# lenskit/csr

Hardware: AMD Instinct MI355X
Metric: spmv_gflops (higher is better)
Workload: dtype f64

## Files before the change

csr_amd/csrc/spmv.hip:

```cpp
#include "spmv_plan.h"

#include <algorithm>
#include <ctime>

namespace csrk {
template <bool R32>
__device__ __forceinline__ double spmv_prod(double a, double x)
{
    const double t = a * x;
    return R32 ? (double)(float)t : t;
}

void free_spmv_plan(SpmvPlan *p) { delete p; }

void spmv_plan_bytes_by_part(const SpmvPlan *p, int64_t out[5])
{
    for (int i = 0; i < 5; i++) out[i] = 0;
    auto add = [&](int part, std::initializer_list<const DevBuf *> bufs) {
        for (const DevBuf *b : bufs) out[part] += (int64_t)b->bytes;
    };
    for (const AccPanel *ap : p->acc) add(0, {&ap->row_list, &ap->vals, &ap->idx, &ap->tile_row0, &ap->segs, &ap->wg_seg, &ap->partial, &ap->z, &ap->wg_map});
    const Panel &t = p->tier1;
    add(1, {&t.row_list, &t.rp, &t.ci, &t.vs, &t.tile, &t.group, &t.carry_row, &t.carry_val, &t.y, &t.crp, &t.cidx});
    const LightStream *l = &p->ls;
// ... 386 lines not shown
                int q = atomicAdd(&s_nlong, 1);
                s_long[q] = r;
                continue;
            }
            double acc = ordered_sum(s_prod, s, e);
            if (r < nr) {
                yp[i0 + r] = acc;
            } else {
                *(pt.cslot >= 0 ? yp + pt.cslot : carry_val + t) = acc;
            }
        }
        __syncthreads();
        const int nlong = s_nlong;
        for (int q = wv; q < nlong; q += PT / WAVE) {
            int r = s_long[q];
            int s = r ? s_rend[r - 1] : 0;
            int e = s_rend[r];
            double acc = 0.0;
            for (int k = s + lane; k < e; k += WAVE) acc += s_prod[k];
            acc = wave_sum(acc);
            if (lane == 0) {
                if (r < nr) {
                    yp[i0 + r] = acc;
                } else {
                    *(pt.cslot >= 0 ? yp + pt.cslot : carry_val + t) = acc;
                }
            }
        }
        pt = nx;
    }
#undef PANEL_LOAD_TILE
}

template <int CB, int PT, bool R32 = false, class SV = double, class XT = double>
__global__ __launch_bounds__(PT) void spmv_acc_kernel(const AccLaunchArgs L, const XT *__restrict__ x, int32_t ncols)
{
    uint32_t grp = 0, wg = blockIdx.x;
    if (L.wg_map) {
        const uint32_t id = L.wg_map[blockIdx.x];
        grp = id >> 16;
        wg = id & 0xffffu;
    }
    const AccGroupArgs &A = L.g[grp];
    const SV *__restrict__ pvals = (const SV *)A.vals;
    const uint16_t *__restrict__ pidx = A.idx;
    const int32_t *__restrict__ tile_row0 = A.tile_row0;
    const AccSeg *__restrict__ segs = A.segs;
    const int32_t *__restrict__ wg_seg = A.wg_seg;
    double *__restrict__ partial = A.partial;
    const int32_t H = A.H;
    const int32_t fx_g = A.fx_g;
    extern __shared__ __align__(16) unsigned char acc_smem[];
    double *s_x = (double *)acc_smem;
    double *s_acc = s_x + CB + 2;
    const int Hpad = (H + 1) & ~1;
    double *s_hval = s_acc + Hpad;
    int32_t *s_hrow = (int32_t *)(s_hval + ACC_SEG_TILES);
    constexpr int NW = PT / WAVE;
    const int tid = threadIdx.x, lane = tid & (WAVE - 1), wv = tid / WAVE;

    for (int h = tid; h < Hpad; h += PT) s_acc[h] = 0.0;
    if (tid < 2) s_x[CB + tid] = 0.0;
    const unsigned long long below = lane ? (~0ull >> (WAVE - lane)) : 0ull;
    const unsigned long long upto = below | (1ull << lane);

    int cur_blk = -1;
    const int sb = wg_seg[wg], se = wg_seg[wg + 1];
    for (int si = sb; si < se; si++) {
        const AccSeg sg = segs[si];
        if (sg.blk != cur_blk) {
            cur_blk = sg.blk;
            const int32_t w0 = sg.blk * CB;
            const int wlen = ncols - w0 < CB ? ncols - w0 : CB;
            if (wlen == CB) {
                constexpr int WL = CB / 2 / PT;
                f64x2_t v[WL];
#pragma unroll
                for (int u = 0; u < WL; u++) {
                    if (sizeof(XT) == 8) {
                        v[u] = *((const F64x2 *)(x + w0) + tid + u * PT);
                    } else {
                        const f32x2_t t = *((const F32x2 *)(x + w0) + tid + u * PT);
                        v[u].x = (double)t.x;
                        v[u].y = (double)t.y;
                    }
                }
#pragma unroll
                for (int u = 0; u < WL; u++) ((f64x2_t *)s_x)[tid + u * PT] = v[u];
            } else {
                for (int k = tid; k < wlen; k += PT) s_x[k] = (double)x[w0 + k];
            }
        }
        __syncthreads();

        const int nt = sg.ntiles;
        AccVals<SV> v, vn;
        u32x4_t ix, ixn;
        int32_t tr0 = 0, tr0n = 0;
        int t = wv;
        const int64_t pstep = (int64_t)A.n_wg;
        if (t < nt) {
            const u32x4_t *ip = (const u32x4_t *)(pidx + (sg.ptile0 + t * pstep) * ACC_TILE);
            v.load(acc_tile_at(pvals, sg.ptile0 + t * pstep), lane);
            ix = __builtin_nontemporal_load(ip + lane);
            tr0 = tile_row0[sg.tile0 + t];
        }
        for (; t < nt; t += NW) {
            const bool more = t + NW < nt;
            if (more) {
                const u32x4_t *ip = (const u32x4_t *)(pidx + (sg.ptile0 + (t + NW) * pstep) * ACC_TILE);
                vn.load(acc_tile_at(pvals, sg.ptile0 + (t + NW) * pstep), lane);
                ixn = __builtin_nontemporal_load(ip + lane);
                tr0n = tile_row0[sg.tile0 + t + NW];
            }
            uint32_t e[ACC_K] = {ix.x & 0xffffu, ix.x >> 16, ix.y & 0xffffu, ix.y >> 16,
                                 ix.z & 0xffffu, ix.z >> 16, ix.w & 0xffffu, ix.w >> 16};
            double a[ACC_K];
            if constexpr (std::is_same<SV, fix56::nib::Bytes>::value) v.get(a, fx_g, e);
            else v.get(a, fx_g);
            double xv[ACC_K];
#pragma unroll
            for (int j = 0; j < ACC_K; j++) xv[j] = s_x[e[j] & ACC_COL_MASK];
            int rw[ACC_K];
            {
                int lsum = 0;
#pragma unroll
                for (int j = 0; j < ACC_K; j++) lsum += (int)(e[j] >> ACC_ROW_SHIFT);
                int run = tr0 + wave_exscan_i32(lsum, lane);
#pragma unroll
                for (int j = 0; j < ACC_K; j++) {
                    run += (int)(e[j] >> ACC_ROW_SHIFT);
                    rw[j] = run;
                }
            }
            const int hr = rw[0];
            int cur = hr;
            double acc = 0.0, hs = 0.0;
            bool nb = false;
#pragma unroll
            for (int j = 0; j < ACC_K; j++) {
                const int r = rw[j];
                if (r != cur) {
                    if (!nb) {
                        hs = acc;
                        nb = true;
                    } else {
                        atomicAdd(&s_acc[cur], acc);
                    }
                    acc = 0.0;
                    cur = r;
                }
                if (R32) acc += spmv_prod<true>(a[j], xv[j]);
                else acc += a[j] * xv[j];
            }
            const int tr = cur;
            const double ts = acc;
            if (!nb) hs = acc;
            const int tr_prev = wave_up1_i32(tr, -1);
            const bool ne = lane > 0 && tr_prev != hr;
            const double T = wave_segscan(ts, nb || ne, lane);
            const double T_prev = wave_up1_f64(T, 0.0);
            const double X = (lane > 0 && !ne) ? T_prev : 0.0;
            const unsigned long long m_nb = __ballot(nb), m_ne = __ballot(ne);
            const bool before = ((m_nb & below) | (m_ne & upto)) != 0;
            const int ne_next = wave_down1_i32((int)ne, 1);
            const bool tail_done = lane == WAVE - 1 || ne_next != 0;
            if (nb) {
                const double hv = hs + X;
                if (before) {
                    atomicAdd(&s_acc[hr], hv);
                } else {
                    s_hrow[t] = hr;
                    s_hval[t] = hv;
                }
            }
            if (tail_done) {
                if (nb || before) {
                    atomicAdd(&s_acc[tr], T);
                } else {
                    s_hrow[t] = tr;
                    s_hval[t] = T;
                }
            }
            if (more) {
                v = vn;
                ix = ixn;
                tr0 = tr0n;
            }
        }
        __syncthreads();
        if (wv == 0) {
            for (int base = 0; base < nt; base += WAVE) {
                const int i = base + lane;
                const bool ok = i < nt;
                const int row = ok ? s_hrow[i] : -1 - lane;
                const double val = ok ? s_hval[i] : 0.0;
                const int row_prev = wave_up1_i32(row, -2 - WAVE);
                const double S = wave_segscan(val, lane == 0 || row_prev != row, lane);
                const int row_next = wave_down1_i32(row, -2 - WAVE);
                if (ok && (lane == WAVE - 1 || row_next != row)) atomicAdd(&s_acc[row], S);
            }
        }
    }
    __syncthreads();
    for (int h = tid; h < H; h += PT) partial[(int64_t)wg * H + h] = s_acc[h];
}

struct EpiJob {
    int32_t kind, blocks;
    const int32_t *carry_row;
    const double *carry_val;
    int64_t n;
    double *fy;
    const double *partial;
    const int32_t *row_list;
    int32_t H, n_wg, G;
    int32_t extra;
    const int32_t *crp, *cidx;
    const double *cval;
};
struct EpiJobs {
    EpiJob j[6];
    int32_t n;
};
constexpr int EPI_THREADS = 1024;

__global__ __launch_bounds__(EPI_THREADS) void spmv_epilogue_kernel(EpiJobs jobs, double *__restrict__ y)
{
    __shared__ double s_p[EPI_THREADS / WAVE][WAVE];
    int b = blockIdx.x, q = 0;
    while (q + 1 < jobs.n && b >= jobs.j[q].blocks) b -= jobs.j[q++].blocks;
    const EpiJob &J = jobs.j[q];
    if (J.kind == 0) {
        const int64_t t = (int64_t)b * EPI_THREADS + threadIdx.x;
// ... 412 lines not shown
    int32_t c[LS_STAGE_IPT], d[LS_STAGE_IPT];
#pragma unroll
    for (int q = 0; q < LS_STAGE_IPT; q++) {
        const int32_t k = k0 + (int32_t)threadIdx.x + q * LS_STAGE_THREADS;
        c[q] = k < k1 ? (int32_t)__builtin_nontemporal_load(a_col + k) : -1;
        d[q] = k < k1 ? __builtin_nontemporal_load(a_dst + k) : 0;
    }
    for (int i = threadIdx.x; i < W; i += LS_STAGE_THREADS) s_x[i] = c0 + i < ncols ? (double)x[c0 + i] : 0.0;
    __syncthreads();
    for (int32_t kb = k0; kb < k1; kb += LS_STAGE_THREADS * LS_STAGE_IPT) {
        int32_t cn[LS_STAGE_IPT], dn[LS_STAGE_IPT];
        const int32_t kn = kb + LS_STAGE_THREADS * LS_STAGE_IPT;
        if (kn < k1) {
#pragma unroll
            for (int q = 0; q < LS_STAGE_IPT; q++) {
                const int32_t k = kn + (int32_t)threadIdx.x + q * LS_STAGE_THREADS;
                cn[q] = k < k1 ? (int32_t)__builtin_nontemporal_load(a_col + k) : -1;
                dn[q] = k < k1 ? __builtin_nontemporal_load(a_dst + k) : 0;
            }
        }
#pragma unroll
        for (int q = 0; q < LS_STAGE_IPT; q++)
            if (c[q] >= 0) xg[d[q]] = s_x[c[q]];
        if (kn < k1) {
#pragma unroll
            for (int q = 0; q < LS_STAGE_IPT; q++) c[q] = cn[q], d[q] = dn[q];
        }
    }
}

int spmv_kernel_attributes()
{
    for (const void *f : {(const void *)spmv_acc_kernel<ACC_CB, ACC_THREADS>, (const void *)spmv_lstream_kernel<LS_PLAIN>,
                          (const void *)spmv_lstream_kernel<LS_RND>, (const void *)spmv_lstream_kernel<LS_PLAIN, true>,
                          (const void *)spmv_lstream_kernel<LS_RND, true>, (const void *)spmv_acc_kernel<ACC_CB, ACC_THREADS, true>,
                          (const void *)spmv_lstream_kernel<LS_PLAIN, false, true>, (const void *)spmv_lstream_kernel<LS_RND, false, true>,
                          (const void *)spmv_lstream_kernel<LS_PLAIN, true, true>, (const void *)spmv_lstream_kernel<LS_RND, true, true>,
                          (const void *)spmv_acc_kernel<ACC_CB, ACC_THREADS, false, float>,
                          (const void *)spmv_acc_kernel<ACC_CB, ACC_THREADS, true, float>,
                          (const void *)spmv_lstream_kernel<LS_PLAIN, false, false, float>, (const void *)spmv_lstream_kernel<LS_RND, false, false, float>,
                          (const void *)spmv_lstream_kernel<LS_PLAIN, true, false, float>, (const void *)spmv_lstream_kernel<LS_RND, true, false, float>,
                          (const void *)spmv_lstream_kernel<LS_PLAIN, false, true, float>, (const void *)spmv_lstream_kernel<LS_RND, false, true, float>,
                          (const void *)spmv_lstream_kernel<LS_PLAIN, true, true, float>, (const void *)spmv_lstream_kernel<LS_RND, true, true, float>,
                          (const void *)spmv_lstream_kernel<LS_RND24>, (const void *)spmv_lstream_kernel<LS_RND24, true>,
                          (const void *)spmv_lstream_kernel<LS_RND24, false, true>, (const void *)spmv_lstream_kernel<LS_RND24, true, true>,
                          (const void *)spmv_lstream_kernel<LS_RND24, false, false, float>, (const void *)spmv_lstream_kernel<LS_RND24, true, false, float>,
                          (const void *)spmv_lstream_kernel<LS_RND24, false, true, float>, (const void *)spmv_lstream_kernel<LS_RND24, true, true, float>,
                          (const void *)spmv_acc_kernel<ACC_CB, ACC_THREADS, false, double, float>,
                          (const void *)spmv_acc_kernel<ACC_CB, ACC_THREADS, true, double, float>,
                          (const void *)spmv_acc_kernel<ACC_CB, ACC_THREADS, false, float, float>,
                          (const void *)spmv_acc_kernel<ACC_CB, ACC_THREADS, true, float, float>,
                          (const void *)spmv_acc_kernel<ACC_CB, ACC_THREADS, false, fix56::Packed>,
                          (const void *)spmv_acc_kernel<ACC_CB, ACC_THREADS, true, fix56::Packed>,
                          (const void *)spmv_acc_kernel<ACC_CB, ACC_THREADS, false, fix56::Packed, float>,
                          (const void *)spmv_acc_kernel<ACC_CB, ACC_THREADS, true, fix56::Packed, float>,
                          (const void *)spmv_acc_kernel<ACC_CB, ACC_THREADS, false, fix56::nib::Bytes>,
                          (const void *)spmv_acc_kernel<ACC_CB, ACC_THREADS, true, fix56::nib::Bytes>,
                          (const void *)spmv_acc_kernel<ACC_CB, ACC_THREADS, false, fix56::nib::Bytes, float>,
                          (const void *)spmv_acc_kernel<ACC_CB, ACC_THREADS, true, fix56::nib::Bytes, float>})
        CSRK_HIP(hipFuncSetAttribute(f, hipFuncAttributeMaxDynamicSharedMemorySize, (int)(160 * 1024)));
    CSRK_HIP(hipFuncSetAttribute((const void *)ls_stage_kernel<double>, hipFuncAttributeMaxDynamicSharedMemorySize, (int)(LS_STAGE_WMAX * 8)));
    CSRK_HIP(hipFuncSetAttribute((const void *)ls_stage_kernel<float>, hipFuncAttributeMaxDynamicSharedMemorySize, (int)(LS_STAGE_WMAX * 8)));
    return CSRK_OK;
}

static int get_plan_locked(Matrix *m, hipStream_t s, SpmvPlan **out, bool launching)
{
    if (launching) m->spmv_calls++;
    const char *env = getenv("CSRK_SPMV_HEAVY_SPLIT"), *env_hot = getenv("CSRK_SPMV_HOT"), *env_ls = getenv("CSRK_SPMV_STREAM");
    const bool eager = (env && env[0] == '1') || (env_hot && env_hot[0] == '1') || (env_ls && env_ls[0] == '1') || !launching;
    const bool want_split = eager || m->spmv_calls >= 2;
    if (m->spmv_plan && !m->spmv_plan->split_considered && want_split && m->spmv_plan->algo == CSRK_SPMV_MERGE &&
        !m->spmv_plan->profiling) {
        if (hipDeviceSynchronize() != hipSuccess) {
            set_error("device synchronisation failed: %s", hipGetErrorString(hipGetLastError()));
            return CSRK_ERR_HIP;
        }
        free_spmv_plan(m->spmv_plan);
        m->spmv_plan = nullptr;
    }
    if (!m->spmv_plan) {
        SpmvPlan *p = new (std::nothrow) SpmvPlan();
        CSRK_REQUIRE(p, "out of host memory");
        p->algo = m->spmv_algo == CSRK_SPMV_AUTO ? CSRK_SPMV_MERGE : m->spmv_algo;
        (void)s;
        int rc = build_spmv_plan(m, p, want_split);
        if (rc == CSRK_OK && hipDeviceSynchronize() != hipSuccess) {
            set_error("SpMV plan construction failed: %s", hipGetErrorString(hipGetLastError()));
            rc = CSRK_ERR_HIP;
        }
        if (rc != CSRK_OK) {
            delete p;
// ... 70 lines not shown
            KernelTimer ks(p, s, 3);
            const unsigned gs = (unsigned)(ceil_div(p->ls.n_stage_blk, 8) * 8);
            ls_stage_kernel<XT><<<gs, LS_STAGE_THREADS, (size_t)p->ls.stage_w * 8, s>>>(
                d_x, m->ncols, p->ls.stage_w, p->ls.a_col.as<uint16_t>(), p->ls.a_dst.as<int32_t>(),
                p->ls.blk_start.as<int32_t>(), p->ls.n_stage_blk, p->ls.xg.as<double>());
            ks.stop();
            CSRK_LAUNCH_CHECK();
        }
        if (do_light && p->n_hot && !(p->ls.on && p->ls.n_cold)) {
            hot_pack_kernel<XT><<<(unsigned)ceil_div(p->n_hot, 256), 256, 0, s>>>(d_x, p->hot_cols.as<int32_t>(), p->n_hot,
                                                                            p->xh.as<double>());
            CSRK_LAUNCH_CHECK();
        }
        bool t0_rides = false;
        if (do_heavy && p->n_heavy && !p->acc.empty()) {
            KernelTimer kh(p, s, 1);
            for (size_t a0 = 0; a0 < p->acc.size(); a0 += (size_t)p->acc[a0]->launch_groups) {
                AccPanel *ap = p->acc[a0];
                const int gb = ap->launch_groups;
                if (gb < 1 || gb > accgroups::MAX_GROUPS || a0 + (size_t)gb > p->acc.size()) {
                    set_error("internal: tier 0's groups and launches disagree");
                    return CSRK_ERR_INVALID;
                }
                AccLaunchArgs L = {};
                size_t lds = 0;
                for (int g = 0; g < gb; g++) {
                    const AccPanel *aq = p->acc[a0 + (size_t)g];
                    L.g[g] = {aq->vals.p, aq->idx.as<uint16_t>(), aq->tile_row0.as<int32_t>(), aq->segs.as<AccSeg>(),
                              aq->wg_seg.as<int32_t>(), aq->partial.as<double>(), aq->nrow, aq->n_wg, aq->fx_g, 0};
                    lds = aq->lds > lds ? aq->lds : lds;
                }
                L.wg_map = gb > 1 ? ap->wg_map.as<uint32_t>() : nullptr;
                const unsigned n_blocks = (unsigned)(gb > 1 ? ap->launch_wgs : ap->n_wg);
#define ACC_LAUNCH(SV) spmv_acc_kernel<ACC_CB, ACC_THREADS, R32, SV, XT><<<n_blocks, ACC_THREADS, lds, s>>>(L, d_x, m->ncols)
                if (ap->f32) ACC_LAUNCH(float);
                else if (ap->nib) ACC_LAUNCH(fix56::nib::Bytes);
                else if (ap->fix56) ACC_LAUNCH(fix56::Packed);
                else ACC_LAUNCH(double);
#undef ACC_LAUNCH
                CSRK_LAUNCH_CHECK();
            }
            kh.stop();
        }
        if (do_heavy && p->n_heavy && p->tier1.on) {
            Panel *pn = &p->tier1;
            KernelTimer kh(p, s, 2);
#define PANEL_ARGS(PP)                                                                                              \
    pn->rp.as<PP>(), pn->ci.as<int32_t>(), pn->vs.as<double>(), d_x, m->ncols, pn->y.as<double>(),                    \
        pn->tile.as<PanelTile>(), pn->group.as<PanelGroup>(), pn->rows, pn->carry_row.as<int32_t>(),                  \
        pn->carry_val.as<double>(), pn->nnz, pn->cb, rider
            PanelRider rider = {};
            rider.first = pn->groups;
            for (int q = 0; q < accgroups::MAX_GROUPS; q++) rider.start[q] = INT32_MAX;
            int64_t rider_wgs = 0;
            if (PANEL_T1 / WAVE == 4 && do_heavy && !p->acc.empty() && (size_t)p->acc[0]->launch_groups == p->acc.size() &&
                p->acc.size() <= (size_t)accgroups::MAX_GROUPS && p->acc[0]->z.p) {
                for (size_t q = 0; q < p->acc.size(); q++) {
                    AccPanel *ap = p->acc[q];
                    rider.partial[q] = ap->partial.as<double>();
                    rider.z[q] = ap->z.as<double>();
                    rider.H[q] = ap->nrow;
                    rider.n_wg[q] = ap->n_wg;
                    rider.start[q] = (int32_t)rider_wgs;
                    rider_wgs += ceil_div(ap->nrow, WAVE);
                }
                t0_rides = true;
            }
// ... 436 lines not shown
        a_tiles += ap->tiles;
        a_rows += ap->nrow;
        a_nnz += ap->nnz;
        a_nb = ap->nb;
    }
    const bool af = !p->acc.empty();
    const int64_t plan_bytes = spmv_plan_bytes(p);
    int64_t part[5];
    spmv_plan_bytes_by_part(p, part);
    const int64_t v[34] = {p->algo == CSRK_SPMV_MERGE ? p->n_tiles : p->n_segs,
                           p->algo == CSRK_SPMV_MERGE ? p->tile_items : VEC_SEG,
                           p->n_heavy, p->algo == CSRK_SPMV_MERGE ? p->nnz_light : m->nnz,
                           a_tiles, a_nb, p->heavy_min, af ? ACC_CB : 0, p->n_heavy ? 2 : 0, a_rows, a_nnz,
                           t1.nrow, t1.rows, t1.nnz, p->tier1_min, t1.cb,
                           p->n_hot, (int64_t)(p->hot_cover * 1e6), af ? 1 : 0, p->hot_slots,
                           p->ls.on ? 1 : 0, p->ls.n_tiles, p->ls.n_runs, p->ls.grid, p->ls.n_cold, plan_bytes,
                           p->ls.round_start.p ? p->ls.stage_tiles : 0,
                           a_wgs, 0, part[0], part[1], part[2], part[3], part[4]};
    for (int i = 0; i < n && i < 34; i++) out[i] = v[i];
    const LightStream &ls = p->ls;
    const bool rnd = ls.on && ls.n_cold && ls.round_start.p;
    const int64_t plain_rounds = ls.on ? ceil_div(ls.n_tiles, LS_THREADS / WAVE) : 0;
    const int64_t w[8] = {ls.on && ls.dense ? 1 : 0,
                          ls.on && ls.idx24 ? 1 : 0,
                          ls.on ? p->n_hot_lds : 0,
                          rnd ? ls.n_rounds : plain_rounds,
                          rnd ? ls.max_wg_rounds : (ls.on ? ceil_div(plain_rounds, (int64_t)ls.grid) : 0),
                          rnd ? ls.n_stage_blk : 0,
                          rnd ? ls.stage_w : 0,
                          ls.on && ls.f32 ? 1 : 0};
    for (int i = 34; i < n && i < 42; i++) out[i] = w[i - 34];
    const int64_t u[6] = {t1.nb, t1.tiles, t1.ncs, t1.listed, t1.groups, t1.pad_groups};
    for (int i = 42; i < n && i < 48; i++) out[i] = u[i - 42];
    return CSRK_OK;
}

int csrk_spmv_stream_limits(int64_t *out, int n)
{
    CSRK_REQUIRE(out && n >= 0, "out is NULL");
    const int64_t v[13] = {ACC_TILE, ACC_K, LS_THREADS / WAVE, LS_SEQ, LS_RID, LS_HOT_LDS, LS_RND_HOT, LS_RND_CAP, LS_RND_MAXTILES,
                           LS_STAGE_WMAX, LS_STAGE_THREADS * LS_STAGE_IPT, TIERB_MIN_DEFAULT, HOT_SLOTS_MAX};
    for (int i = 0; i < n && i < 13; i++) out[i] = v[i];
    return CSRK_OK;
}


int csrk_spmv_plan_info(csrk_handle_t h, int64_t *n_tiles, int32_t *tile_items)
{
    Matrix *m = from_handle(h);
    if (!m) return CSRK_ERR_INVALID;
    SpmvPlan *p = nullptr;
    CSRK_TRY(get_plan(m, nullptr, &p));
    if (n_tiles) *n_tiles = p->algo == CSRK_SPMV_MERGE ? p->n_tiles : p->n_segs;
    if (tile_items) *tile_items = p->algo == CSRK_SPMV_MERGE ? p->tile_items : VEC_SEG;
    return CSRK_OK;
}

}
```

csr_amd/csrc/spmv_plan.h:

```cpp
#pragma once
#include "common.h"
#include "device_loads.h"
#include "wave.h"
#include "fix56.h"
#include "acc_groups.h"

#include <type_traits>
#include <vector>

namespace csrk {

__device__ __forceinline__ double wave_sum(double v)
{
#pragma unroll
    for (int off = WAVE / 2; off > 0; off >>= 1) v += __shfl_down(v, off, WAVE);
    return v;
}

__device__ __forceinline__ double ordered_sum(const double *p, int s, int e)
{
    double acc = 0.0;
    int k = s;
    for (; k + 4 <= e; k += 4) {
        const double a = p[k], b = p[k + 1], c = p[k + 2], d = p[k + 3];
        acc += a;
        acc += b;
        acc += c;
        acc += d;
    }
    for (; k < e; k++) acc += p[k];
    return acc;
}

struct Panel {
    bool on = false, p64 = false;
    int32_t cb = 0, nb = 0, nrow = 0;
    int64_t rows = 0, tiles = 0, nnz = 0, groups = 0;
    DevBuf row_list;
    DevBuf rp, ci, vs, tile, group, carry_row, carry_val, y;
    int32_t ncs = 0;
    DevBuf crp, cidx;
    int64_t listed = 0, pad_groups = 0;
};

struct AccSeg {
    int64_t tile0;
    int64_t ptile0;
    int32_t ntiles;
    int32_t blk;
};

struct AccPanel {
    int32_t nrow = 0, nb = 0, n_wg = 0;
    int32_t launch_groups = 1, launch_wgs = 0;
    DevBuf wg_map;
    int64_t tiles = 0, nnz = 0, n_segs = 0;
    size_t lds = 0;
    DevBuf row_list, vals, idx, tile_row0, segs, wg_seg, partial;
    DevBuf z;
    bool f32 = false;
    bool fix56 = false;
    bool nib = false;
    int32_t fx_g = 0;
};

struct LightStream {
    bool on = false;
    int64_t n_tiles = 0;
    int32_t n_runs = 0, n_out = 0;
    unsigned grid = 0;
    DevBuf vals, idx, rowids, tile_base, carry_row, carry_val;
    bool idx24 = false;
    bool f32 = false;
    bool dense = false;
    int64_t n_cold = 0;
    int32_t n_stage_blk = 0, stage_w = 0;
    DevBuf xg, a_col, a_dst, blk_start;
    int32_t stage_tiles = 0;
    int32_t n_rounds = 0, max_wg_rounds = 0;
    DevBuf round_start, round_tile0, wg_round0;
};

struct SpmvPlan {
    int algo = CSRK_SPMV_MERGE;
    int tile_items = 0;
    int64_t n_tiles = 0;
    DevBuf tile_row;
    DevBuf carry_row;
    DevBuf carry_val;
// ... 289 lines not shown
```

csr_amd/csrc/spmv_plan.hip:

```cpp
#include "spmv_plan.h"

#include <algorithm>
#include <cstring>
#include <ctime>
#include <type_traits>

namespace csrk {
struct PlanTrace {
    bool on;
    double t0;
    static double now()
    {
        timespec ts;
        clock_gettime(CLOCK_MONOTONIC, &ts);
        return ts.tv_sec * 1e3 + ts.tv_nsec * 1e-6;
    }
    PlanTrace() : on(getenv("CSRK_PLAN_TRACE") != nullptr), t0(0.0)
    {
        if (on) {
            (void)hipDeviceSynchronize();
            t0 = now();
        }
    }
    void lap(const char *what)
// ... 941 lines not shown
        }
    const int64_t n_tasks = (int64_t)trow.size();
    CSRK_TRY(pstart.alloc((size_t)(pairs + n) * 4));
    CSRK_TRY(d_trow.alloc((size_t)(n_tasks ? n_tasks : 1) * 4));
    CSRK_TRY(d_tpiece.alloc((size_t)(n_tasks ? n_tasks : 1) * 4));
    CSRK_TRY(stage_h2d(d_trow.p, trow.data(), (size_t)n_tasks * 4, s));
    CSRK_TRY(stage_h2d(d_tpiece.p, tpiece.data(), (size_t)n_tasks * 4, s));
    acc_pairstart_kernel<P><<<(unsigned)(ceil_div(ceil_div(n_tasks * WAVE, 256), 8) * 8), 256, 0, s>>>(
        rp, m->d_colinds, ap->row_list.as<int32_t>(), n, nb, ACC_CB, d_trow.as<int32_t>(), d_tpiece.as<int32_t>(), n_tasks,
        pstart.as<int32_t>());
    CSRK_LAUNCH_CHECK();
    tr.lap("  tier 0: pair starts");
    acc_paircount_kernel<<<(unsigned)ceil_div(pairs, 256), 256, 0, s>>>(pstart.as<int32_t>(), pairs, n, off.as<int64_t>());
    CSRK_LAUNCH_CHECK();
    DevBuf gap;
    CSRK_TRY(gap.alloc((size_t)pairs * 4));
    acc_gap_kernel<<<(unsigned)ceil_div((int64_t)nb * WAVE, 256), 256, 0, s>>>(off.as<int64_t>(), n, nb, gap.as<int32_t>());
    CSRK_LAUNCH_CHECK();
    CSRK_TRY(exclusive_scan_i64(off.as<int64_t>(), off.as<int64_t>(), pairs, s));
    CSRK_TRY(bends.alloc((size_t)(nb + 1) * 8));
    panel_blockends_kernel<<<(unsigned)ceil_div(nb + 1, 256), 256, 0, s>>>(off.as<int64_t>(), n, nb, bends.as<int64_t>());
    CSRK_LAUNCH_CHECK();
    std::vector<int64_t> be((size_t)nb + 1), t0((size_t)nb + 1);
    CSRK_TRY(stage_d2h(be.data(), bends.p, (size_t)(nb + 1) * 8, s));
    CSRK_HIP(hipStreamSynchronize(s));
    t0[0] = 0;
    for (int32_t b = 0; b < nb; b++) t0[b + 1] = t0[b] + ceil_div(be[b + 1] - be[b], ACC_TILE);
    const int64_t n_tiles = t0[nb];
    CSRK_TRY(stage_h2d(bends.p, t0.data(), (size_t)(nb + 1) * 8, s));
    tr.lap("  tier 0: counts, gaps, scan");
    int cus = 0;
    CSRK_HIP(hipDeviceGetAttribute(&cus, hipDeviceAttributeMultiprocessorCount, m->device));
    int64_t n_wg = wg_want > 0 ? wg_want : cus > 0 ? cus : 256;
    if (n_wg > n_tiles) n_wg = n_tiles;
    if (n_wg < 1) n_wg = 1;
    std::vector<int64_t> wg_t0((size_t)n_wg + 1);
    int64_t share_max = 0;
    for (int64_t w = 0; w <= n_wg; w++) wg_t0[(size_t)w] = n_tiles * w / n_wg;
    for (int64_t w = 0; w < n_wg; w++) share_max = std::max(share_max, wg_t0[(size_t)w + 1] - wg_t0[(size_t)w]);
    const int64_t n_phys = share_max * n_wg;
    DevBuf d_wg_t0;
    CSRK_TRY(d_wg_t0.alloc((size_t)(n_wg + 1) * 8));
    CSRK_TRY(stage_h2d(d_wg_t0.p, wg_t0.data(), (size_t)(n_wg + 1) * 8, s));
    ap->f32 = VT == CSRK_VAL_F32;
    DevBuf fx;
    CSRK_TRY(fx.alloc(16));
    if (VT == CSRK_VAL_F64 && n > 0 && form != ACC_FORM_RAW) {
        const char *env = getenv("CSRK_SPMV_FIX56");
        if (!(env && env[0] == '0')) {
            int32_t h[4] = {0, INT32_MAX, INT32_MIN, 0};
            CSRK_TRY(stage_h2d(fx.p, h, sizeof h, s));
            acc_range_kernel<P><<<dim3((unsigned)n, 16), 256, 0, s>>>(rp, (const double *)m->d_values, ap->row_list.as<int32_t>(),
                                                                     fx.as<int32_t>());
            CSRK_LAUNCH_CHECK();
            CSRK_TRY(stage_d2h(h, fx.p, sizeof h, s));
            CSRK_HIP(hipStreamSynchronize(s));
            fix56::Range r;
            r.bad = h[0];
            r.lo = h[1];
            r.hi = h[2];
            ap->fix56 = fix56::packable(r, ap->fx_g);
            ap->nib = ap->fix56 && form == ACC_FORM_NIB;
            tr.lap("  tier 0: value grid test");
        }
    }
    CSRK_TRY(ap->idx.alloc((size_t)n_phys * ACC_TILE * 2));
// ... 48 lines not shown
    for (int64_t w = 0; w < n_wg; w++) {
        wg_seg[(size_t)w] = (int32_t)segs.size();
        int64_t t = wg_t0[(size_t)w];
        const int64_t t_end = wg_t0[(size_t)w + 1];
        while (t < t_end) {
            while (t0[b + 1] <= t) b++;
            int64_t e = t_end < t0[b + 1] ? t_end : t0[b + 1];
            if (e - t > ACC_SEG_TILES) e = t + ACC_SEG_TILES;
            AccSeg sg;
            sg.tile0 = t;
            sg.ptile0 = (t - wg_t0[(size_t)w]) * n_wg + w;
            sg.ntiles = (int32_t)(e - t);
            sg.blk = b;
            segs.push_back(sg);
            t = e;
        }
    }
    wg_seg[(size_t)n_wg] = (int32_t)segs.size();
    CSRK_TRY(ap->segs.alloc(segs.size() * sizeof(AccSeg)));
    CSRK_TRY(ap->wg_seg.alloc(wg_seg.size() * 4));
    CSRK_TRY(stage_h2d(ap->segs.p, segs.data(), segs.size() * sizeof(AccSeg), s));
    CSRK_TRY(stage_h2d(ap->wg_seg.p, wg_seg.data(), wg_seg.size() * 4, s));
    CSRK_TRY(ap->partial.alloc((size_t)n_wg * n * 8));
    CSRK_TRY(ap->z.alloc((size_t)n * 8));
    ap->lds = (size_t)(ACC_CB + 2) * 8 + (size_t)((n + 1) & ~1) * 8 + (size_t)ACC_SEG_TILES * 12;
    CSRK_TRY(spmv_kernel_attributes());
    CSRK_HIP(hipStreamSynchronize(s));
    ap->nrow = n;
    ap->nb = nb;
    ap->n_wg = (int32_t)n_wg;
    ap->tiles = n_tiles;
    ap->nnz = nnz_rows;
    ap->n_segs = (int64_t)segs.size();
    if (tr.on)
        fprintf(stderr, "[csrk plan]   tier 0 group: rows %d entries %lld workgroups %lld tiles %lld, %.1f per segment%s\n", n,
                (long long)nnz_rows, (long long)n_wg, (long long)n_tiles, segs.empty() ? 0.0 : (double)n_tiles / (double)segs.size(),
                ap->nib ? " (nib)" : ap->fix56 ? " (fix56)" : ap->f32 ? " (float32)" : " (raw)");
    tr.lap("  tier 0: segments");
    return CSRK_OK;
}

static int acc_nib_knob()
{
    const char *env = getenv("CSRK_SPMV_NIB");
    if (!env || !env[0]) return -1;
    return env[0] == '0' ? 0 : 1;
}

static int acc_groups_knob()
{
    const char *e = getenv("CSRK_ACC_GROUPS");
    const int g = e ? atoi(e) : ACC_GROUPS_DEFAULT;
    return g < 1 ? 1 : g > accgroups::MAX_GROUPS ? accgroups::MAX_GROUPS : g;
}
static int32_t acc_group_rows_knob()
{
    const char *e = getenv("CSRK_ACC_GROUP_ROWS");
    const int r = e ? atoi(e) : ACC_MAXROWS;
    return r < 1 || r > ACC_MAXROWS ? ACC_MAXROWS : r;
}


template <class P>
static int build_heavy_split(Matrix *m, SpmvPlan *p, hipStream_t s, bool allow_tier1 = true)
{
    p->n_heavy = 0;
// ... 840 lines not shown
```

Baseline: 835.6.

## Pipeline tile and x-window prefetch across segments in accumulate SpMV kernel

Adds a pipelined variant of the accumulate kernel that prefetches the next segment's first tile and the next x window into registers while the current segment is still being reduced. Segment descriptors are read through a uniform (scalar) address space. This is meant to hide the global-load latency at segment boundaries that the old loop exposed after each barrier. The variant is on by default behind an env switch. It adds register pressure from holding the staged x window and doubles the number of template instantiations.

```diff
diff --git a/csr_amd/csrc/spmv.hip b/csr_amd/csrc/spmv.hip
--- a/csr_amd/csrc/spmv.hip
+++ b/csr_amd/csrc/spmv.hip
@@ -442,7 +442,97 @@
 #undef PANEL_LOAD_TILE
 }
 
-template <int CB, int PT, bool R32 = false, class SV = double, class XT = double>
+template <bool R32, class SV>
+__device__ __forceinline__ void acc_tile_reduce(const AccVals<SV> &v, const u32x4_t ix, const int tr0, const int32_t fx_g,
+                                                const double *s_x, double *s_acc, int32_t *s_hrow, double *s_hval, const int t,
+                                                const int lane, const unsigned long long below, const unsigned long long upto)
+{
+    uint32_t e[ACC_K] = {ix.x & 0xffffu, ix.x >> 16, ix.y & 0xffffu, ix.y >> 16,
+                         ix.z & 0xffffu, ix.z >> 16, ix.w & 0xffffu, ix.w >> 16};
+    double a[ACC_K];
+    if constexpr (std::is_same<SV, fix56::nib::Bytes>::value) v.get(a, fx_g, e);
+    else v.get(a, fx_g);
+    double xv[ACC_K];
+#pragma unroll
+    for (int j = 0; j < ACC_K; j++) xv[j] = s_x[e[j] & ACC_COL_MASK];
+    int rw[ACC_K];
+    {
+        int lsum = 0;
+#pragma unroll
+        for (int j = 0; j < ACC_K; j++) lsum += (int)(e[j] >> ACC_ROW_SHIFT);
+        int run = tr0 + wave_exscan_i32(lsum, lane);
+#pragma unroll
+        for (int j = 0; j < ACC_K; j++) {
+            run += (int)(e[j] >> ACC_ROW_SHIFT);
+            rw[j] = run;
+        }
+    }
+    const int hr = rw[0];
+    int cur = hr;
+    double acc = 0.0, hs = 0.0;
+    bool nb = false;
+#pragma unroll
+    for (int j = 0; j < ACC_K; j++) {
+        const int r = rw[j];
+        if (r != cur) {
+            if (!nb) {
+                hs = acc;
+                nb = true;
+            } else {
+                atomicAdd(&s_acc[cur], acc);
+            }
+            acc = 0.0;
+            cur = r;
+        }
+        if (R32) acc += spmv_prod<true>(a[j], xv[j]);
+        else acc += a[j] * xv[j];
+    }
+    const int tr = cur;
+    const double ts = acc;
+    if (!nb) hs = acc;
+    const int tr_prev = wave_up1_i32(tr, -1);
+    const bool ne = lane > 0 && tr_prev != hr;
+    const double T = wave_segscan(ts, nb || ne, lane);
+    const double T_prev = wave_up1_f64(T, 0.0);
+    const double X = (lane > 0 && !ne) ? T_prev : 0.0;
+    const unsigned long long m_nb = __ballot(nb), m_ne = __ballot(ne);
+    const bool before = ((m_nb & below) | (m_ne & upto)) != 0;
+    const int ne_next = wave_down1_i32((int)ne, 1);
+    const bool tail_done = lane == WAVE - 1 || ne_next != 0;
+    if (nb) {
+        const double hv = hs + X;
+        if (before) {
+            atomicAdd(&s_acc[hr], hv);
+        } else {
+            s_hrow[t] = hr;
+            s_hval[t] = hv;
+        }
+    }
+    if (tail_done) {
+        if (nb || before) {
+            atomicAdd(&s_acc[tr], T);
+        } else {
+            s_hrow[t] = tr;
+            s_hval[t] = T;
+        }
+    }
+}
+
+__device__ __forceinline__ AccSeg acc_seg_uniform(const AccSeg *segs, int i)
+{
+    typedef const int64_t __attribute__((address_space(4))) *C64;
+    typedef const int32_t __attribute__((address_space(4))) *C32;
+    static_assert(sizeof(AccSeg) == 24, "two 64-bit words, two 32-bit words");
+    const uintptr_t at = (uintptr_t)(segs + i);
+    AccSeg sg;
+    sg.tile0 = ((C64)at)[0];
+    sg.ptile0 = ((C64)at)[1];
+    sg.ntiles = ((C32)at)[4];
+    sg.blk = ((C32)at)[5];
+    return sg;
+}
+
+template <int CB, int PT, bool R32 = false, class SV = double, class XT = double, bool PIPE = false>
 __global__ __launch_bounds__(PT) void spmv_acc_kernel(const AccLaunchArgs L, const XT *__restrict__ x, int32_t ncols)
 {
     uint32_t grp = 0, wg = blockIdx.x;
@@ -474,142 +564,164 @@
     const unsigned long long below = lane ? (~0ull >> (WAVE - lane)) : 0ull;
     const unsigned long long upto = below | (1ull << lane);
 
-    int cur_blk = -1;
-    const int sb = wg_seg[wg], se = wg_seg[wg + 1];
-    for (int si = sb; si < se; si++) {
-        const AccSeg sg = segs[si];
-        if (sg.blk != cur_blk) {
-            cur_blk = sg.blk;
-            const int32_t w0 = sg.blk * CB;
+    auto fold_heads = [&](const int nt) {
+        for (int base = 0; base < nt; base += WAVE) {
+            const int i = base + lane;
+            const bool ok = i < nt;
+            const int row = ok ? s_hrow[i] : -1 - lane;
+            const double val = ok ? s_hval[i] : 0.0;
+            const int row_prev = wave_up1_i32(row, -2 - WAVE);
+            const double S = wave_segscan(val, lane == 0 || row_prev != row, lane);
+            const int row_next = wave_down1_i32(row, -2 - WAVE);
+            if (ok && (lane == WAVE - 1 || row_next != row)) atomicAdd(&s_acc[row], S);
+        }
+    };
+    if constexpr (PIPE) {
+        const int wvu = __builtin_amdgcn_readfirstlane(wv);
+        const int sb = __builtin_amdgcn_readfirstlane(wg_seg[wg]), se = __builtin_amdgcn_readfirstlane(wg_seg[wg + 1]);
+        const int64_t pstep = (int64_t)A.n_wg;
+        constexpr int WL = CB / 2 / PT;
+        static_assert(WL * 2 * PT == CB, "a window is WL pairs per thread");
+        typedef typename std::conditional<sizeof(XT) == 8, f64x2_t, f32x2_t>::type X2;
+        typedef typename std::conditional<sizeof(XT) == 8, F64x2, F32x2>::type X2U;
+        X2 wr[WL];
+        auto window_request = [&](const int blk) {
+            const int32_t w0 = blk * CB;
             const int wlen = ncols - w0 < CB ? ncols - w0 : CB;
             if (wlen == CB) {
-                constexpr int WL = CB / 2 / PT;
-                f64x2_t v[WL];
+#pragma unroll
+                for (int u = 0; u < WL; u++) wr[u] = *((const X2U *)(x + w0) + tid + u * PT);
+            } else {
 #pragma unroll
                 for (int u = 0; u < WL; u++) {
-                    if (sizeof(XT) == 8) {
-                        v[u] = *((const F64x2 *)(x + w0) + tid + u * PT);
-                    } else {
-                        const f32x2_t t = *((const F32x2 *)(x + w0) + tid + u * PT);
-                        v[u].x = (double)t.x;
-                        v[u].y = (double)t.y;
+                    const int k0 = tid + 2 * u * PT, k1 = k0 + PT;
+                    wr[u].x = x[w0 + (k0 < wlen ? k0 : wlen - 1)];
+                    wr[u].y = x[w0 + (k1 < wlen ? k1 : wlen - 1)];
+                }
+            }
+        };
+        auto window_store = [&](const int blk) {
+            const int32_t w0 = blk * CB;
+            const int wlen = ncols - w0 < CB ? ncols - w0 : CB;
+            if (wlen == CB) {
+#pragma unroll
+                for (int u = 0; u < WL; u++) {
+                    f64x2_t d;
+                    d.x = (double)wr[u].x;
+                    d.y = (double)wr[u].y;
+                    ((f64x2_t *)s_x)[tid + u * PT] = d;
+                }
+            } else {
+#pragma unroll
+                for (int u = 0; u < WL; u++) {
+                    const int k0 = tid + 2 * u * PT, k1 = k0 + PT;
+                    if (k0 < wlen) s_x[k0] = (double)wr[u].x;
+                    if (k1 < wlen) s_x[k1] = (double)wr[u].y;
+                }
+            }
+        };
+        AccVals<SV> v, vn;
+        u32x4_t ix = {0, 0, 0, 0}, ixn;
+        int32_t tr0 = 0, tr0n;
+        auto tile_request = [&](AccVals<SV> &dv, u32x4_t &dix, int32_t &dtr, const int64_t ptile, const int64_t ltile) {
+            dv.load(acc_tile_at(pvals, ptile), lane);
+            dix = __builtin_nontemporal_load((const u32x4_t *)(pidx + ptile * ACC_TILE) + lane);
+            dtr = tile_row0[ltile];
+        };
+        if (sb < se) {
+            AccSeg sg = acc_seg_uniform(segs, sb);
+            window_request(sg.blk);
+            if (wvu < sg.ntiles) tile_request(v, ix, tr0, sg.ptile0 + wvu * pstep, sg.tile0 + wvu);
+            bool fill = true;
+            for (int si = sb; si < se; si++) {
+                const bool has_next = si + 1 < se;
+                const AccSeg nx = acc_seg_uniform(segs, has_next ? si + 1 : si);
+                if (fill) window_store(sg.blk);
+                __syncthreads();
+                const int nt = sg.ntiles;
+                const bool next_mine = has_next && wvu < nx.ntiles;
+                const int64_t pt_first = nx.ptile0 + wvu * pstep, lt_first = nx.tile0 + wvu;
+                const bool fill_next = has_next && nx.blk != sg.blk;
+                if (wvu >= nt) {
+                    if (next_mine) tile_request(v, ix, tr0, pt_first, lt_first);
+                    if (fill_next) window_request(nx.blk);
+                }
+                for (int t = wvu; t < nt; t += NW) {
+                    const bool more = t + NW < nt;
+                    const int64_t pt_n = more ? sg.ptile0 + (t + NW) * pstep : next_mine ? pt_first : sg.ptile0 + t * pstep;
+                    const int64_t lt_n = more ? sg.tile0 + t + NW : next_mine ? lt_first : sg.tile0 + t;
+                    tile_request(vn, ixn, tr0n, pt_n, lt_n);
+                    if (!more && fill_next) window_request(nx.blk);
+                    acc_tile_reduce<R32, SV>(v, ix, tr0, fx_g, s_x, s_acc, s_hrow, s_hval, t, lane, below, upto);
+                    v = vn;
+                    ix = ixn;
+                    tr0 = tr0n;
+                }
+                __syncthreads();
+                if (wv == 0) fold_heads(nt);
+                fill = fill_next;
+                sg = nx;
+            }
+        }
+    } else {
+        int cur_blk = -1;
+        const int sb = wg_seg[wg], se = wg_seg[wg + 1];
+        for (int si = sb; si < se; si++) {
+            const AccSeg sg = segs[si];
+            if (sg.blk != cur_blk) {
+                cur_blk = sg.blk;
+                const int32_t w0 = sg.blk * CB;
+                const int wlen = ncols - w0 < CB ? ncols - w0 : CB;
+                if (wlen == CB) {
+                    constexpr int WL = CB / 2 / PT;
+                    f64x2_t v[WL];
+#pragma unroll
+                    for (int u = 0; u < WL; u++) {
+                        if (sizeof(XT) == 8) {
+                            v[u] = *((const F64x2 *)(x + w0) + tid + u * PT);
+                        } else {
+                            const f32x2_t t = *((const F32x2 *)(x + w0) + tid + u * PT);
+                            v[u].x = (double)t.x;
+                            v[u].y = (double)t.y;
+                        }
                     }
+#pragma unroll
+                    for (int u = 0; u < WL; u++) ((f64x2_t *)s_x)[tid + u * PT] = v[u];
+                } else {
+                    for (int k = tid; k < wlen; k += PT) s_x[k] = (double)x[w0 + k];
                 }
-#pragma unroll
-                for (int u = 0; u < WL; u++) ((f64x2_t *)s_x)[tid + u * PT] = v[u];
-            } else {
-                for (int k = tid; k < wlen; k += PT) s_x[k] = (double)x[w0 + k];
-            }
-        }
-        __syncthreads();
-
-        const int nt = sg.ntiles;
-        AccVals<SV> v, vn;
-        u32x4_t ix, ixn;
-        int32_t tr0 = 0, tr0n = 0;
-        int t = wv;
-        const int64_t pstep = (int64_t)A.n_wg;
-        if (t < nt) {
-            const u32x4_t *ip = (const u32x4_t *)(pidx + (sg.ptile0 + t * pstep) * ACC_TILE);
-            v.load(acc_tile_at(pvals, sg.ptile0 + t * pstep), lane);
-            ix = __builtin_nontemporal_load(ip + lane);
-            tr0 = tile_row0[sg.tile0 + t];
-        }
-        for (; t < nt; t += NW) {
-            const bool more = t + NW < nt;
-            if (more) {
-                const u32x4_t *ip = (const u32x4_t *)(pidx + (sg.ptile0 + (t + NW) * pstep) * ACC_TILE);
-                vn.load(acc_tile_at(pvals, sg.ptile0 + (t + NW) * pstep), lane);
-                ixn = __builtin_nontemporal_load(ip + lane);
-                tr0n = tile_row0[sg.tile0 + t + NW];
-            }
-            uint32_t e[ACC_K] = {ix.x & 0xffffu, ix.x >> 16, ix.y & 0xffffu, ix.y >> 16,
-                                 ix.z & 0xffffu, ix.z >> 16, ix.w & 0xffffu, ix.w >> 16};
-            double a[ACC_K];
-            if constexpr (std::is_same<SV, fix56::nib::Bytes>::value) v.get(a, fx_g, e);
-            else v.get(a, fx_g);
-            double xv[ACC_K];
-#pragma unroll
-            for (int j = 0; j < ACC_K; j++) xv[j] = s_x[e[j] & ACC_COL_MASK];
-            int rw[ACC_K];
-            {
-                int lsum = 0;
-#pragma unroll
-                for (int j = 0; j < ACC_K; j++) lsum += (int)(e[j] >> ACC_ROW_SHIFT);
-                int run = tr0 + wave_exscan_i32(lsum, lane);
-#pragma unroll
-                for (int j = 0; j < ACC_K; j++) {
-                    run += (int)(e[j] >> ACC_ROW_SHIFT);
-                    rw[j] = run;
+            }
+            __syncthreads();
+
+            const int nt = sg.ntiles;
+            AccVals<SV> v, vn;
+            u32x4_t ix, ixn;
+            int32_t tr0 = 0, tr0n = 0;
+            int t = wv;
+            const int64_t pstep = (int64_t)A.n_wg;
+            if (t < nt) {
+                const u32x4_t *ip = (const u32x4_t *)(pidx + (sg.ptile0 + t * pstep) * ACC_TILE);
+                v.load(acc_tile_at(pvals, sg.ptile0 + t * pstep), lane);
+                ix = __builtin_nontemporal_load(ip + lane);
+                tr0 = tile_row0[sg.tile0 + t];
+            }
+            for (; t < nt; t += NW) {
+                const bool more = t + NW < nt;
+                if (more) {
+                    const u32x4_t *ip = (const u32x4_t *)(pidx + (sg.ptile0 + (t + NW) * pstep) * ACC_TILE);
+                    vn.load(acc_tile_at(pvals, sg.ptile0 + (t + NW) * pstep), lane);
+                    ixn = __builtin_nontemporal_load(ip + lane);
+                    tr0n = tile_row0[sg.tile0 + t + NW];
                 }
-            }
-            const int hr = rw[0];
-            int cur = hr;
-            double acc = 0.0, hs = 0.0;
-            bool nb = false;
-#pragma unroll
-            for (int j = 0; j < ACC_K; j++) {
-                const int r = rw[j];
-                if (r != cur) {
-                    if (!nb) {
-                        hs = acc;
-                        nb = true;
-                    } else {
-                        atomicAdd(&s_acc[cur], acc);
-                    }
-                    acc = 0.0;
-                    cur = r;
+                acc_tile_reduce<R32, SV>(v, ix, tr0, fx_g, s_x, s_acc, s_hrow, s_hval, t, lane, below, upto);
+                if (more) {
+                    v = vn;
+                    ix = ixn;
+                    tr0 = tr0n;
                 }
-                if (R32) acc += spmv_prod<true>(a[j], xv[j]);
-                else acc += a[j] * xv[j];
-            }
-            const int tr = cur;
-            const double ts = acc;
-            if (!nb) hs = acc;
-            const int tr_prev = wave_up1_i32(tr, -1);
-            const bool ne = lane > 0 && tr_prev != hr;
-            const double T = wave_segscan(ts, nb || ne, lane);
-            const double T_prev = wave_up1_f64(T, 0.0);
-            const double X = (lane > 0 && !ne) ? T_prev : 0.0;
-            const unsigned long long m_nb = __ballot(nb), m_ne = __ballot(ne);
-            const bool before = ((m_nb & below) | (m_ne & upto)) != 0;
-            const int ne_next = wave_down1_i32((int)ne, 1);
-            const bool tail_done = lane == WAVE - 1 || ne_next != 0;
-            if (nb) {
-                const double hv = hs + X;
-                if (before) {
-                    atomicAdd(&s_acc[hr], hv);
-                } else {
-                    s_hrow[t] = hr;
-                    s_hval[t] = hv;
-                }
-            }
-            if (tail_done) {
-                if (nb || before) {
-                    atomicAdd(&s_acc[tr], T);
-                } else {
-                    s_hrow[t] = tr;
-                    s_hval[t] = T;
-                }
-            }
-            if (more) {
-                v = vn;
-                ix = ixn;
-                tr0 = tr0n;
-            }
-        }
-        __syncthreads();
-        if (wv == 0) {
-            for (int base = 0; base < nt; base += WAVE) {
-                const int i = base + lane;
-                const bool ok = i < nt;
-                const int row = ok ? s_hrow[i] : -1 - lane;
-                const double val = ok ? s_hval[i] : 0.0;
-                const int row_prev = wave_up1_i32(row, -2 - WAVE);
-                const double S = wave_segscan(val, lane == 0 || row_prev != row, lane);
-                const int row_next = wave_down1_i32(row, -2 - WAVE);
-                if (ok && (lane == WAVE - 1 || row_next != row)) atomicAdd(&s_acc[row], S);
-            }
+            }
+            __syncthreads();
+            if (wv == 0) fold_heads(nt);
         }
     }
     __syncthreads();
@@ -1088,12 +1200,16 @@
 int spmv_kernel_attributes()
 {
     for (const void *f : {(const void *)spmv_acc_kernel<ACC_CB, ACC_THREADS>, (const void *)spmv_lstream_kernel<LS_PLAIN>,
+                          (const void *)spmv_acc_kernel<ACC_CB, ACC_THREADS, false, double, double, true>,
+                          (const void *)spmv_acc_kernel<ACC_CB, ACC_THREADS, true, double, double, true>,
                           (const void *)spmv_lstream_kernel<LS_RND>, (const void *)spmv_lstream_kernel<LS_PLAIN, true>,
                           (const void *)spmv_lstream_kernel<LS_RND, true>, (const void *)spmv_acc_kernel<ACC_CB, ACC_THREADS, true>,
                           (const void *)spmv_lstream_kernel<LS_PLAIN, false, true>, (const void *)spmv_lstream_kernel<LS_RND, false, true>,
                           (const void *)spmv_lstream_kernel<LS_PLAIN, true, true>, (const void *)spmv_lstream_kernel<LS_RND, true, true>,
                           (const void *)spmv_acc_kernel<ACC_CB, ACC_THREADS, false, float>,
+                          (const void *)spmv_acc_kernel<ACC_CB, ACC_THREADS, false, float, double, true>,
                           (const void *)spmv_acc_kernel<ACC_CB, ACC_THREADS, true, float>,
+                          (const void *)spmv_acc_kernel<ACC_CB, ACC_THREADS, true, float, double, true>,
                           (const void *)spmv_lstream_kernel<LS_PLAIN, false, false, float>, (const void *)spmv_lstream_kernel<LS_RND, false, false, float>,
                           (const void *)spmv_lstream_kernel<LS_PLAIN, true, false, float>, (const void *)spmv_lstream_kernel<LS_RND, true, false, float>,
                           (const void *)spmv_lstream_kernel<LS_PLAIN, false, true, float>, (const void *)spmv_lstream_kernel<LS_RND, false, true, float>,
@@ -1103,17 +1219,29 @@
                           (const void *)spmv_lstream_kernel<LS_RND24, false, false, float>, (const void *)spmv_lstream_kernel<LS_RND24, true, false, float>,
                           (const void *)spmv_lstream_kernel<LS_RND24, false, true, float>, (const void *)spmv_lstream_kernel<LS_RND24, true, true, float>,
                           (const void *)spmv_acc_kernel<ACC_CB, ACC_THREADS, false, double, float>,
+                          (const void *)spmv_acc_kernel<ACC_CB, ACC_THREADS, false, double, float, true>,
                           (const void *)spmv_acc_kernel<ACC_CB, ACC_THREADS, true, double, float>,
+                          (const void *)spmv_acc_kernel<ACC_CB, ACC_THREADS, true, double, float, true>,
                           (const void *)spmv_acc_kernel<ACC_CB, ACC_THREADS, false, float, float>,
+                          (const void *)spmv_acc_kernel<ACC_CB, ACC_THREADS, false, float, float, true>,
                           (const void *)spmv_acc_kernel<ACC_CB, ACC_THREADS, true, float, float>,
+                          (const void *)spmv_acc_kernel<ACC_CB, ACC_THREADS, true, float, float, true>,
                           (const void *)spmv_acc_kernel<ACC_CB, ACC_THREADS, false, fix56::Packed>,
+                          (const void *)spmv_acc_kernel<ACC_CB, ACC_THREADS, false, fix56::Packed, double, true>,
                           (const void *)spmv_acc_kernel<ACC_CB, ACC_THREADS, true, fix56::Packed>,
+                          (const void *)spmv_acc_kernel<ACC_CB, ACC_THREADS, true, fix56::Packed, double, true>,
                           (const void *)spmv_acc_kernel<ACC_CB, ACC_THREADS, false, fix56::Packed, float>,
+                          (const void *)spmv_acc_kernel<ACC_CB, ACC_THREADS, false, fix56::Packed, float, true>,
                           (const void *)spmv_acc_kernel<ACC_CB, ACC_THREADS, true, fix56::Packed, float>,
+                          (const void *)spmv_acc_kernel<ACC_CB, ACC_THREADS, true, fix56::Packed, float, true>,
                           (const void *)spmv_acc_kernel<ACC_CB, ACC_THREADS, false, fix56::nib::Bytes>,
+                          (const void *)spmv_acc_kernel<ACC_CB, ACC_THREADS, false, fix56::nib::Bytes, double, true>,
                           (const void *)spmv_acc_kernel<ACC_CB, ACC_THREADS, true, fix56::nib::Bytes>,
+                          (const void *)spmv_acc_kernel<ACC_CB, ACC_THREADS, true, fix56::nib::Bytes, double, true>,
                           (const void *)spmv_acc_kernel<ACC_CB, ACC_THREADS, false, fix56::nib::Bytes, float>,
-                          (const void *)spmv_acc_kernel<ACC_CB, ACC_THREADS, true, fix56::nib::Bytes, float>})
+                          (const void *)spmv_acc_kernel<ACC_CB, ACC_THREADS, false, fix56::nib::Bytes, float, true>,
+                          (const void *)spmv_acc_kernel<ACC_CB, ACC_THREADS, true, fix56::nib::Bytes, float>,
+                          (const void *)spmv_acc_kernel<ACC_CB, ACC_THREADS, true, fix56::nib::Bytes, float, true>})
         CSRK_HIP(hipFuncSetAttribute(f, hipFuncAttributeMaxDynamicSharedMemorySize, (int)(160 * 1024)));
     CSRK_HIP(hipFuncSetAttribute((const void *)ls_stage_kernel<double>, hipFuncAttributeMaxDynamicSharedMemorySize, (int)(LS_STAGE_WMAX * 8)));
     CSRK_HIP(hipFuncSetAttribute((const void *)ls_stage_kernel<float>, hipFuncAttributeMaxDynamicSharedMemorySize, (int)(LS_STAGE_WMAX * 8)));
@@ -1250,7 +1378,11 @@
                 }
                 L.wg_map = gb > 1 ? ap->wg_map.as<uint32_t>() : nullptr;
                 const unsigned n_blocks = (unsigned)(gb > 1 ? ap->launch_wgs : ap->n_wg);
-#define ACC_LAUNCH(SV) spmv_acc_kernel<ACC_CB, ACC_THREADS, R32, SV, XT><<<n_blocks, ACC_THREADS, lds, s>>>(L, d_x, m->ncols)
+#define ACC_LAUNCH(SV)                                                                                                       \
+    do {                                                                                                                     \
+        if (ap->pipe) spmv_acc_kernel<ACC_CB, ACC_THREADS, R32, SV, XT, true><<<n_blocks, ACC_THREADS, lds, s>>>(L, d_x, m->ncols); \
+        else spmv_acc_kernel<ACC_CB, ACC_THREADS, R32, SV, XT, false><<<n_blocks, ACC_THREADS, lds, s>>>(L, d_x, m->ncols);  \
+    } while (0)
                 if (ap->f32) ACC_LAUNCH(float);
                 else if (ap->nib) ACC_LAUNCH(fix56::nib::Bytes);
                 else if (ap->fix56) ACC_LAUNCH(fix56::Packed);
@@ -1753,6 +1885,14 @@
     for (int i = 34; i < n && i < 42; i++) out[i] = w[i - 34];
     const int64_t u[6] = {t1.nb, t1.tiles, t1.ncs, t1.listed, t1.groups, t1.pad_groups};
     for (int i = 42; i < n && i < 48; i++) out[i] = u[i - 42];
+    int64_t a_segs = 0, a_wg_segs = 0, a_min_tiles = 0;
+    for (const AccPanel *ap : p->acc) {
+        if (ap->n_segs) a_min_tiles = a_segs ? std::min<int64_t>(a_min_tiles, ap->min_seg_tiles) : ap->min_seg_tiles;
+        a_segs += ap->n_segs;
+        a_wg_segs = std::max<int64_t>(a_wg_segs, ap->max_wg_segs);
+    }
+    const int64_t sg3[3] = {a_segs, a_wg_segs, a_min_tiles};
+    for (int i = 48; i < n && i < 51; i++) out[i] = sg3[i - 48];
     return CSRK_OK;
 }
 
diff --git a/csr_amd/csrc/spmv_plan.h b/csr_amd/csrc/spmv_plan.h
--- a/csr_amd/csrc/spmv_plan.h
+++ b/csr_amd/csrc/spmv_plan.h
@@ -55,6 +55,8 @@
     int32_t launch_groups = 1, launch_wgs = 0;
     DevBuf wg_map;
     int64_t tiles = 0, nnz = 0, n_segs = 0;
+    int32_t max_wg_segs = 0, min_seg_tiles = 0;
+    bool pipe = true;
     size_t lds = 0;
     DevBuf row_list, vals, idx, tile_row0, segs, wg_seg, partial;
     DevBuf z;
diff --git a/csr_amd/csrc/spmv_plan.hip b/csr_amd/csrc/spmv_plan.hip
--- a/csr_amd/csrc/spmv_plan.hip
+++ b/csr_amd/csrc/spmv_plan.hip
@@ -997,6 +997,8 @@
     int cus = 0;
     CSRK_HIP(hipDeviceGetAttribute(&cus, hipDeviceAttributeMultiprocessorCount, m->device));
     int64_t n_wg = wg_want > 0 ? wg_want : cus > 0 ? cus : 256;
+    if (const char *e = getenv("CSRK_ACC_WGS"))
+        if (atoi(e) > 0 && n_wg > atoi(e)) n_wg = atoi(e);
     if (n_wg > n_tiles) n_wg = n_tiles;
     if (n_wg < 1) n_wg = 1;
     std::vector<int64_t> wg_t0((size_t)n_wg + 1);
@@ -1111,6 +1113,14 @@
     ap->tiles = n_tiles;
     ap->nnz = nnz_rows;
     ap->n_segs = (int64_t)segs.size();
+    ap->max_wg_segs = 0;
+    for (int64_t w = 0; w < n_wg; w++) ap->max_wg_segs = std::max(ap->max_wg_segs, wg_seg[(size_t)w + 1] - wg_seg[(size_t)w]);
+    ap->min_seg_tiles = segs.empty() ? 0 : INT32_MAX;
+    for (const AccSeg &sg : segs) ap->min_seg_tiles = std::min(ap->min_seg_tiles, sg.ntiles);
+    {
+        const char *env = getenv("CSRK_SPMV_ACC_PIPE");
+        ap->pipe = !(env && env[0] == '0');
+    }
     if (tr.on)
         fprintf(stderr, "[csrk plan]   tier 0 group: rows %d entries %lld workgroups %lld tiles %lld, %.1f per segment%s\n", n,
                 (long long)nnz_rows, (long long)n_wg, (long long)n_tiles, segs.empty() ? 0.0 : (double)n_tiles / (double)segs.size(),
```

New measurement: 842.9 (median of 6 runs). Within noise of the previous version (+0.9%).
